# tanishqkumar/ssd

Hardware: NVIDIA H100
Metric: decode tokens/sec (sync speculative decoding, accept-len reported) (higher is better)
Workload: dtype bf16

## Files before the change

ssd_b200/csrc/draft_stream.cuh:

```cuda
#pragma once
#include "common.cuh"
#include "sampling.cuh"

namespace ssdk {

constexpr int kDsConsumers = 256;
constexpr int kDsWarps = kDsConsumers / 32;
constexpr int kDsThreads = kDsConsumers + 32;
constexpr int kDsMaxLayers = 32;
constexpr int kDsSplits = 16;
constexpr int kDsShortSplits = 8;
constexpr int kDsLongCtx = 256;
constexpr int kDsSlotBytes = 32768;
constexpr int kDsMaxSlots = 6;
constexpr int kDsMaxSteps = 8;
constexpr int kDsBtSmem = 32;

struct DsLayer {
  const __nv_bfloat16 *qkv, *o, *gate_up, *down, *in_norm, *post_norm, *q_norm, *k_norm;
};

struct DsParams {
  int d, L, H, KV, ffn, vocab, qk_norm;
  float eps, scale_log2;
  const __nv_bfloat16 *embed, *final_norm, *lm_head;
  const float* rope;
  __nv_bfloat16 *k_cache, *v_cache;
  long long cache_layer_stride;
  int block_size, max_blocks;
  int64_t* tok_buf;
  int n_fwd;
  int skip_last_head;
  const int32_t* ctx0;
  const int32_t* block_table;
  __nv_bfloat16 *vec_qkv, *vec_attn, *vec_o, *vec_act, *vec_down, *resid0, *resid1;
  float* attn_part;
  __nv_bfloat16* logits;
  long long logits_ld;
  const float* temp;
  const uint64_t* dyn;
  uint64_t seed, call_base;
  ArgMax* samp_partial;
  unsigned* bar_state;
  unsigned* attn_ticket;
  int n_slots;
  DsLayer layers[kDsMaxLayers];
  const int64_t* pend_tok;
  __nv_bfloat16* vec_row0;
};

struct DsVecs {
  __nv_bfloat16 *qkv, *attn, *o, *down, *resid0, *resid1, *act;
  SSDK_DEVINL __nv_bfloat16* resid(int i) const { return i ? resid1 : resid0; }
};
SSDK_DEVINL DsVecs ds_row0_vecs(const DsParams& p, int hd) {
  DsVecs v{};
  __nv_bfloat16* b = p.vec_row0;
  if (!b) return v;
  v.qkv = b; b += ((p.H + 2 * p.KV) * hd + 7) / 8 * 8;
  v.attn = b; b += p.H * hd;
  v.o = b; b += p.d;
  v.down = b; b += p.d;
  v.resid0 = b; b += p.d;
  v.resid1 = b; b += p.d;
  v.act = b;
  return v;
}
__host__ SSDK_DEVINL int ds_xs_floats(int d, int ffn, int q_width) {
  const int a = 2 * d > ffn ? 2 * d : ffn;
  return a > q_width ? a : q_width;
}

SSDK_DEVINL void ds_sync() {
#ifdef SSDK_HOST_EMU
  ::emu::named_barrier(1, kDsConsumers);
#else
  asm volatile("bar.sync 1, 256;" ::: "memory");
#endif
}

struct DsGridBar {
  unsigned long long* counter;
  unsigned long long target;
  __device__ void init() {
    if (threadIdx.x == 0) {
      const unsigned long long c = ld_relaxed_gpu_u64(counter);
      target = c - c % (unsigned long long)gridDim.x;
    }
  }
  __device__ void sync() {
    ds_sync();
    if (threadIdx.x == 0) {
      target += (unsigned long long)gridDim.x;
      red_add_release_gpu_u64(counter, 1ull);
      const long long t0 = clock64();
      while (ld_relaxed_gpu_u64(counter) < target) {
        if (clock64() - t0 > 4000000000LL) __trap();
      }
      fence_acq_rel_gpu();
    }
    ds_sync();
  }
};

SSDK_DEVINL uint4 ds_ldcg16(const void* p) { return __ldcg(reinterpret_cast<const uint4*>(p)); }
SSDK_DEVINL float2 ds_bf2(uint32_t w) { return __bfloat1622float2(*reinterpret_cast<const __nv_bfloat162*>(&w)); }

SSDK_DEVINL void ds_mark(int f, int point) {
  if (f == 1 && threadIdx.x == 0) trace_mark(64 + point);
}

enum { DS_QKV = 0, DS_O = 1, DS_GU = 2, DS_DOWN = 3, DS_HEAD = 4 };
enum { DS_PLAIN = 0, DS_PAIR = 1, DS_SPLIT = 2 };
struct DsGeom {
  int K;
  int rows;
  int kind;
  int rpj;
  int segs;
  int nj;
};
__host__ SSDK_DEVINL bool ds_geometry(int K, int rows, bool pair, DsGeom* g) {
  g->K = K; g->rows = rows; g->segs = 1;
  if (K < 256 || K > 8192 || (K % 256) != 0) return false;
  if (pair) {
    if (K > 2048) return false;
    g->kind = DS_PAIR; g->rpj = 8;
  } else if (K <= 2048) {
    g->kind = DS_PLAIN; g->rpj = 8;
  } else {
    g->kind = DS_SPLIT; g->rpj = K <= 4096 ? 4 : 2; g->segs = kDsWarps / g->rpj;
    if ((K % (256 * g->segs)) != 0) return false;
  }
  g->nj = (rows + g->rpj - 1) / g->rpj;
  return true;
}
SSDK_DEVINL bool ds_has_head(const DsParams& p, int f) { return !(p.skip_last_head && f == p.n_fwd - 1); }
SSDK_DEVINL const __nv_bfloat16* ds_weight(const DsParams& p, int l, int m) {
  const DsLayer& lw = p.layers[l < p.L ? l : 0];
  return m == DS_QKV ? lw.qkv : (m == DS_O ? lw.o : (m == DS_GU ? lw.gate_up : (m == DS_DOWN ? lw.down : p.lm_head)));
}

struct DsCursor {
  int f, l, m, s;
  bool valid;
};
SSDK_DEVINL void ds_cursor_settle(const DsParams& p, const DsGeom* geom, DsCursor& c) {
  while (c.valid && c.s >= geom[c.m].nj) {
    c.s = (int)blockIdx.x;
    if (c.m == DS_HEAD) {
      c.f++; c.l = 0; c.m = DS_QKV;
    } else if (c.m == DS_DOWN) {
      c.l++; c.m = DS_QKV;
      if (c.l == p.L) {
        if (ds_has_head(p, c.f)) c.m = DS_HEAD;
        else { c.f++; c.l = 0; }
      }
    } else {
      c.m++;
    }
    if (c.f >= p.n_fwd) c.valid = false;
  }
// ... 201 lines not shown
  for (int s = (int)blockIdx.x; s < g.nj; s += (int)gridDim.x, ++it) {
    const uint8_t* st = ds_acquire(ring, 0);
    const float acc = ds_dot_seg(st + w_off, steps, lane, xr);
    float acc0 = 0.f;
    if constexpr (TWO) acc0 = ds_dot_seg0(st + w_off, steps, lane, x0 + seg * seg_len);
    ds_release(ring, 0, lane);
    ring.taken += 1u;
    float* rb = res + (it & 1u) * kDsWarps;
    float* rb0 = rb + 2 * kDsWarps;
    if (lane == 0) {
      rb[warp] = acc;
      if constexpr (TWO) rb0[warp] = acc0;
    }
    ds_sync();
    if ((int)threadIdx.x < g.rpj) {
      const int row = s * g.rpj + (int)threadIdx.x;
      if (row < g.rows) {
        float v = 0.f;
        for (int q = 0; q < g.segs; ++q) v += rb[(int)threadIdx.x * g.segs + q];
        y[row] = f2bf(v);
        if constexpr (TWO) {
          float v0 = 0.f;
          for (int q = 0; q < g.segs; ++q) v0 += rb0[(int)threadIdx.x * g.segs + q];
          r0.y[row] = f2bf(v0);
        }
      }
    }
  }
}
SSDK_DEVINL void ds_consume(DsRing& ring, const DsGeom& g, float* xs, float* res, __nv_bfloat16* y, bool two,
                            const DsRow0& r0) {
  if (g.kind == DS_PLAIN) {
    if (two) ds_consume_plain<false, true>(ring, g, xs, y, nullptr, r0);
    else ds_consume_plain<false>(ring, g, xs, y, nullptr);
  } else {
    if (two) ds_consume_split<true>(ring, g, xs, res, y, r0);
    else ds_consume_split<false>(ring, g, xs, res, y, r0);
  }
}
SSDK_DEVINL void ds_consume_gu(DsRing& ring, const DsGeom& g, float* xs, __nv_bfloat16* act, bool two, const DsRow0& r0) {
  if (two) ds_consume_pair<true>(ring, g, xs, act, r0);
  else ds_consume_pair<false>(ring, g, xs, act, r0);
}

SSDK_DEVINL float ds_block_sum(float v, float* red) {
  const int lane = threadIdx.x & 31, wid = threadIdx.x >> 5;
  v = warp_sum(v);
  ds_sync();
  if (lane == 0) red[wid] = v;
  ds_sync();
  float t = (lane < kDsWarps) ? red[lane] : 0.f;
  return warp_sum(t);
}

struct DsPre {
  uint4 w, b;
};
SSDK_DEVINL DsPre ds_preload(const __nv_bfloat16* b, const __nv_bfloat16* w, int d) {
  DsPre r;
  const int i = threadIdx.x * 8;
  r.w = r.b = make_uint4(0u, 0u, 0u, 0u);
  if (i < d) {
    r.w = *reinterpret_cast<const uint4*>(w + i);
    if (b) r.b = ds_ldcg16(b + i);
  }
  return r;
}
SSDK_DEVINL void ds_norm_prologue(const __nv_bfloat16* a, const __nv_bfloat16* b, __nv_bfloat16* resid_out,
                                  const __nv_bfloat16* w, float eps, int d, float* xs, float* red, const DsPre* pre) {
  float ss = 0.f;
  const int i0 = threadIdx.x * 8;
  for (int i = i0; i < d; i += kDsConsumers * 8) {
    float x[8];
    unpack_bf16x8(ds_ldcg16(a + i), x);
    if (b) {
      float y[8];
      unpack_bf16x8((pre && i == i0) ? pre->b : ds_ldcg16(b + i), y);
#pragma unroll
      for (int j = 0; j < 8; ++j) x[j] += y[j];
    }
    if (resid_out && blockIdx.x == 0) *reinterpret_cast<uint4*>(resid_out + i) = pack_bf16x8(x);
#pragma unroll
    for (int j = 0; j < 8; ++j) {
      xs[i + j] = x[j];
      ss += x[j] * x[j];
    }
  }
  ss = ds_block_sum(ss, red);
  const float rstd = rsqrtf(ss / (float)d + eps);
  for (int i = i0; i < d; i += kDsConsumers * 8) {
    float wv[8];
    unpack_bf16x8((pre && i == i0) ? pre->w : *reinterpret_cast<const uint4*>(w + i), wv);
#pragma unroll
    for (int j = 0; j < 8; ++j) xs[i + j] = bf16_round(xs[i + j] * rstd * wv[j]);
  }
  ds_sync();
}
SSDK_DEVINL void ds_load_vec(const __nv_bfloat16* v, int n, float* xs) {
  for (int i = threadIdx.x * 8; i < n; i += kDsConsumers * 8) {
    float x[8];
    unpack_bf16x8(ds_ldcg16(v + i), x);
#pragma unroll
    for (int j = 0; j < 8; ++j) xs[i + j] = x[j];
  }
  ds_sync();
}

SSDK_DEVINL int ds_num_splits(int ctx) {
  return ctx > kDsLongCtx ? kDsSplits : min(kDsShortSplits, max(1, (ctx + 7) >> 3));
}
SSDK_DEVINL int ds_page_of(const DsParams& p, const int* bt_s, int t) {
  const int i = t / p.block_size;
  return p.max_blocks <= kDsBtSmem ? bt_s[i] : p.block_table[i];
}
template <int HD, int TB>
SSDK_DEVINL void ds_load_kv(const DsParams& p, const int* bt_s, const __nv_bfloat16* kbase, const __nv_bfloat16* vbase, int h,
                            int tb, int t1, int pos, int lane, float (&kv)[TB][HD / 32], float (&vv)[TB][HD / 32]) {
  constexpr int EPL = HD / 32;
  static_assert(EPL == 2 || EPL == 4, "head_dim 64 or 128");
#pragma unroll
  for (int u = 0; u < TB; ++u) {
    const int t = tb + u * kDsWarps;
#pragma unroll
    for (int e = 0; e < EPL; ++e) kv[u][e] = vv[u][e] = 0.f;
    if (t < t1 && t != pos) {
      const int blk = ds_page_of(p, bt_s, t);
      const size_t off = (((size_t)blk * p.block_size + t % p.block_size) * p.KV + h) * HD + lane * EPL;
      if constexpr (EPL == 2) {
        const float2 a = ds_bf2(__ldcg(reinterpret_cast<const uint32_t*>(kbase + off)));
        const float2 b = ds_bf2(__ldcg(reinterpret_cast<const uint32_t*>(vbase + off)));
        kv[u][0] = a.x; kv[u][1] = a.y; vv[u][0] = b.x; vv[u][1] = b.y;
      } else {
        const uint2 a = __ldcg(reinterpret_cast<const uint2*>(kbase + off));
        const uint2 b = __ldcg(reinterpret_cast<const uint2*>(vbase + off));
        float2 f = ds_bf2(a.x); kv[u][0] = f.x; kv[u][1] = f.y;
        f = ds_bf2(a.y); kv[u][EPL - 2] = f.x; kv[u][EPL - 1] = f.y;
        f = ds_bf2(b.x); vv[u][0] = f.x; vv[u][1] = f.y;
        f = ds_bf2(b.y); vv[u][EPL - 2] = f.x; vv[u][EPL - 1] = f.y;
      }
    }
  }
}
template <int HD, int GMAX, int TB>
SSDK_DEVINL void ds_attention_unit(const DsParams& p, const __nv_bfloat16* vqkv, __nv_bfloat16* vattn, int layer, int h,
                                   int s, int ns, int ctx, float* sm, int* flag, const int* bt_s) {
  constexpr int HALF = HD / 2;
  constexpr int EPL = HD / 32;
  const int warp = threadIdx.x >> 5, lane = threadIdx.x & 31;
  const int G = p.H / p.KV;
  const int pos = ctx - 1;
  float* sq = sm;
  float* sk = sq + GMAX * HD;
  float* sv = sk + HD;
  float* sred = sv + HD;

  const int per = (ctx + ns - 1) / ns;
  const int t0 = s * per, t1 = min(ctx, t0 + per);
  const __nv_bfloat16* kbase = p.k_cache + (size_t)layer * p.cache_layer_stride;
  const __nv_bfloat16* vbase = p.v_cache + (size_t)layer * p.cache_layer_stride;
  float kv[TB][EPL], vv[TB][EPL];
  ds_load_kv<HD, TB>(p, bt_s, kbase, vbase, h, t0 + warp, t1, pos, lane, kv, vv);

  const float* cs = p.rope + (size_t)pos * HD;
  for (int row = warp; row < G + 2; row += kDsWarps) {
    const int kind = row < G ? 0 : (row == G ? 1 : 2);
    const int col0 = (kind == 0 ? (h * G + row) : (kind == 1 ? p.H + h : p.H + p.KV + h)) * HD;
    float x1[(HALF + 31) / 32], x2[(HALF + 31) / 32];
    float ss = 0.f;
#pragma unroll
    for (int t = 0; t < (HALF + 31) / 32; ++t) {
      const int i = lane + 32 * t;
      x1[t] = x2[t] = 0.f;
      if (i < HALF) {
        const unsigned short a = __ldcg(reinterpret_cast<const unsigned short*>(vqkv + col0 + i));
        const unsigned short b = __ldcg(reinterpret_cast<const unsigned short*>(vqkv + col0 + HALF + i));
        x1[t] = __bfloat162float(__ushort_as_bfloat16(a));
        x2[t] = __bfloat162float(__ushort_as_bfloat16(b));
        ss += x1[t] * x1[t] + x2[t] * x2[t];
      }
    }
    float* dst = kind == 0 ? sq + row * HD : (kind == 1 ? sk : sv);
    if (kind == 2) {
#pragma unroll
      for (int t = 0; t < (HALF + 31) / 32; ++t) {
        const int i = lane + 32 * t;
        if (i < HALF) {
          dst[i] = x1[t];
          dst[HALF + i] = x2[t];
        }
      }
      continue;
    }
    const __nv_bfloat16* nw = p.qk_norm ? (kind == 0 ? p.layers[layer].q_norm : p.layers[layer].k_norm) : nullptr;
    if (nw) {
      ss = warp_sum(ss);
      const float rstd = rsqrtf(ss / (float)HD + p.eps);
#pragma unroll
      for (int t = 0; t < (HALF + 31) / 32; ++t) {
        const int i = lane + 32 * t;
        if (i < HALF) {
          x1[t] = bf16_round(x1[t] * rstd * bf2f(nw[i]));
          x2[t] = bf16_round(x2[t] * rstd * bf2f(nw[HALF + i]));
        }
      }
    }
#pragma unroll
    for (int t = 0; t < (HALF + 31) / 32; ++t) {
      const int i = lane + 32 * t;
      if (i < HALF) {
        const float c = cs[i], sn = cs[HALF + i];
        dst[i] = bf16_round(x1[t] * c - x2[t] * sn);
        dst[HALF + i] = bf16_round(x2[t] * c + x1[t] * sn);
      }
    }
  }
  ds_sync();

  const int blk_new = ds_page_of(p, bt_s, pos);
  if (s == 0 && blk_new >= 0) {
    const size_t slot = (size_t)blk_new * p.block_size + pos % p.block_size;
    __nv_bfloat16* kc = p.k_cache + (size_t)layer * p.cache_layer_stride + (slot * p.KV + h) * HD;
    __nv_bfloat16* vc = p.v_cache + (size_t)layer * p.cache_layer_stride + (slot * p.KV + h) * HD;
    for (int i = threadIdx.x; i < HD; i += kDsConsumers) {
      kc[i] = f2bf(sk[i]);
      vc[i] = f2bf(sv[i]);
    }
  }

  float qreg[GMAX][EPL];
#pragma unroll
  for (int g = 0; g < GMAX; ++g)
#pragma unroll
    for (int e = 0; e < EPL; ++e) qreg[g][e] = (g < G) ? sq[g * HD + lane * EPL + e] : 0.f;
  float m[GMAX], l[GMAX], acc[GMAX][EPL];
#pragma unroll
  for (int g = 0; g < GMAX; ++g) {
    m[g] = -INFINITY;
    l[g] = 0.f;
#pragma unroll
    for (int e = 0; e < EPL; ++e) acc[g][e] = 0.f;
  }
  for (int tb = t0 + warp; tb < t1; tb += TB * kDsWarps) {
    if (tb != t0 + warp) ds_load_kv<HD, TB>(p, bt_s, kbase, vbase, h, tb, t1, pos, lane, kv, vv);
#pragma unroll
    for (int u = 0; u < TB; ++u) {
      const int t = tb + u * kDsWarps;
      if (t < t1) {
        if (t == pos) {
#pragma unroll
          for (int e = 0; e < EPL; ++e) {
            kv[u][e] = sk[lane * EPL + e];
            vv[u][e] = sv[lane * EPL + e];
          }
        }
#pragma unroll
        for (int g = 0; g < GMAX; ++g) {
          if (g < G) {
            float sc = 0.f;
#pragma unroll
            for (int e = 0; e < EPL; ++e) sc = fmaf(qreg[g][e], kv[u][e], sc);
            sc = warp_sum(sc) * p.scale_log2;
            const float mn = fmaxf(m[g], sc);
            const float corr = exp2f(m[g] - mn);
            const float pr = exp2f(sc - mn);
            l[g] = l[g] * corr + pr;
#pragma unroll
            for (int e = 0; e < EPL; ++e) acc[g][e] = acc[g][e] * corr + pr * vv[u][e];
            m[g] = mn;
          }
        }
      }
    }
  }
  constexpr int LDR = HD + 2;
#pragma unroll
  for (int g = 0; g < GMAX; ++g) {
    if (g < G) {
      float* w = sred + ((size_t)warp * G + g) * LDR;
#pragma unroll
      for (int e = 0; e < EPL; ++e) w[lane * EPL + e] = acc[g][e];
      if (lane == 0) {
        w[HD] = m[g];
        w[HD + 1] = l[g];
      }
    }
  }
  ds_sync();
  for (int idx = threadIdx.x; idx < G * HD; idx += kDsConsumers) {
    const int g = idx / HD, dim = idx - g * HD;
    float mx = -INFINITY;
    for (int w = 0; w < kDsWarps; ++w) mx = fmaxf(mx, sred[((size_t)w * G + g) * LDR + HD]);
    float o = 0.f, ll = 0.f;
    if (mx != -INFINITY) {
      for (int w = 0; w < kDsWarps; ++w) {
        const float* r = sred + ((size_t)w * G + g) * LDR;
        const float wt = exp2f(r[HD] - mx);
        o += r[dim] * wt;
        ll += r[HD + 1] * wt;
      }
    }
    if (ns == 1) {
      vattn[(size_t)(h * G + g) * HD + dim] = f2bf(ll > 0.f ? o / ll : 0.f);
    } else {
      float* out = p.attn_part + ((size_t)(h * G + g) * kDsSplits + s) * LDR;
      out[dim] = o;
      if (dim == 0) {
        out[HD] = mx;
        out[HD + 1] = ll;
      }
    }
  }
  if (ns == 1) {
    ds_sync();
    return;
  }
  ds_sync();
  if (threadIdx.x == 0) *flag = (atom_add_acq_rel_gpu(p.attn_ticket + h, 1u) == (unsigned)ns - 1u) ? 1 : 0;
  ds_sync();
  if (*flag) {
    if (threadIdx.x == 0) st_relaxed_gpu_u32(p.attn_ticket + h, 0u);
    for (int idx = threadIdx.x; idx < G * HD; idx += kDsConsumers) {
      const int g = idx / HD, dim = idx - g * HD;
      const float* base = p.attn_part + (size_t)(h * G + g) * kDsSplits * LDR;
      float ms[kDsSplits], ls[kDsSplits], os[kDsSplits];
      float mx = -INFINITY;
#pragma unroll
      for (int q = 0; q < kDsSplits; ++q) {
        const bool on = q < ns;
        ms[q] = on ? __ldcg(base + q * LDR + HD) : -INFINITY;
        ls[q] = on ? __ldcg(base + q * LDR + HD + 1) : 0.f;
        os[q] = on ? __ldcg(base + q * LDR + dim) : 0.f;
        mx = fmaxf(mx, ms[q]);
      }
      float o = 0.f, l = 0.f;
#pragma unroll
      for (int q = 0; q < kDsSplits; ++q) {
        const float wt = (ms[q] == -INFINITY) ? 0.f : exp2f(ms[q] - mx);
        o += os[q] * wt;
        l += ls[q] * wt;
      }
      vattn[(size_t)(h * G + g) * HD + dim] = f2bf(l > 0.f ? o / l : 0.f);
    }
  }
  ds_sync();
}


template <int HD, int GMAX>
__global__ void __launch_bounds__(kDsThreads, 1) draft_stream_kernel(const __grid_constant__ DsParams p) {
  SSDK_DYN_SMEM(uint8_t, ds_smem);
  SSDK_STATIC_SMEM(uint64_t, full_bar, kDsMaxSlots);
  SSDK_STATIC_SMEM(uint64_t, empty_bar, kDsMaxSlots);
  SSDK_STATIC_SMEM(DsGeom, geom, 5);
  SSDK_STATIC_SMEM(float, red, 32);
  SSDK_STATIC_SMEM(float, res, 4 * kDsWarps);
  SSDK_STATIC_SMEM(ArgMax, ared, 32);
  SSDK_SHARED_VAR(int, tok_s);
  SSDK_SHARED_VAR(int, flag_s);
  SSDK_STATIC_SMEM(int, bt_s, kDsBtSmem);
  float* xs = reinterpret_cast<float*>(ds_smem + (size_t)p.n_slots * kDsSlotBytes);
  float* scratch = xs + ds_xs_floats(p.d, p.ffn, p.H * HD);
  if (threadIdx.x < kDsBtSmem && (int)threadIdx.x < p.max_blocks) bt_s[threadIdx.x] = p.block_table[threadIdx.x];
  if (threadIdx.x == 0) {
    trace_mark(TR_MISC);
    ds_geometry(p.d, (p.H + 2 * p.KV) * HD, false, &geom[DS_QKV]);
    ds_geometry(p.H * HD, p.d, false, &geom[DS_O]);
    ds_geometry(p.d, p.ffn, true, &geom[DS_GU]);
    ds_geometry(p.ffn, p.d, false, &geom[DS_DOWN]);
    ds_geometry(p.d, p.vocab, false, &geom[DS_HEAD]);
    for (int s = 0; s < p.n_slots; ++s) {
      mbar_init(&full_bar[s], 1);
      mbar_init(&empty_bar[s], kDsWarps);
    }
    fence_mbar_init();
  }
  __syncthreads();

  if (threadIdx.x >= kDsConsumers) {
    if (threadIdx.x == kDsConsumers) ds_producer(p, geom, ds_smem, full_bar, empty_bar);
    return;
  }

  DsRing ring;
  ring.base = ds_smem;
  ring.full = full_bar;
  ring.empty = empty_bar;
  ring.n_slots = (unsigned)p.n_slots;
  ring.taken = 0u;
  DsGridBar bar;
  bar.counter = reinterpret_cast<unsigned long long*>(p.bar_state);
  bar.target = 0;
  bar.init();

  const int ctx_base = p.ctx0[0];
  const float T = p.temp ? p.temp[0] : 0.f;
  const uint64_t seed = p.dyn ? p.dyn[0] : p.seed;
  const uint64_t call0 = p.dyn ? p.dyn[1] * 16ull : p.call_base;
  __nv_bfloat16* resid[2] = {p.resid0, p.resid1};
  long long tok = p.tok_buf[0];
  const long long tok0 = p.pend_tok ? p.pend_tok[0] : -1;
  const DsVecs v0 = ds_row0_vecs(p, HD);

  for (int f = 0; f < p.n_fwd; ++f) {
    if (threadIdx.x == 0 && f > 0) trace_mark(TR_MISC);
    const int ctx = ctx_base + f + 1;
    const __nv_bfloat16* emb = p.embed + (size_t)tok * p.d;
    const bool two = f == 0 && tok0 >= 0;
    int cur = 0;
    DsPre pre;
    for (int l = 0; l < p.L; ++l) {
      const DsLayer& lw = p.layers[l];
      if (l == 0) {
        if (two) ds_norm_prologue(p.embed + (size_t)tok0 * p.d, nullptr, v0.resid(cur ^ 1), lw.in_norm, p.eps, p.d, xs + p.d, red,
                                  nullptr);
        ds_norm_prologue(emb, nullptr, resid[cur ^ 1], lw.in_norm, p.eps, p.d, xs, red, nullptr);
      } else {
        if (two) ds_norm_prologue(v0.down, v0.resid(cur), v0.resid(cur ^ 1), lw.in_norm, p.eps, p.d, xs + p.d, red, nullptr);
        ds_norm_prologue(p.vec_down, resid[cur], resid[cur ^ 1], lw.in_norm, p.eps, p.d, xs, red, &pre);
      }
      cur ^= 1;
      ds_mark(f, 0);
      ds_consume(ring, geom[DS_QKV], xs, res, p.vec_qkv, two, DsRow0{xs + p.d, nullptr, v0.qkv});
      ds_mark(f, 1);
      bar.sync();
      ds_mark(f, 2);
#ifdef SSDK_TRACE_FINE
      bar.sync();
      ds_mark(f, 12);
#endif
      if (two) {
        const int ns0 = ds_num_splits(ctx - 1);
        for (int u = blockIdx.x; u < p.KV * ns0; u += gridDim.x) {
          if (ns0 == kDsSplits)
            ds_attention_unit<HD, GMAX, 8>(p, v0.qkv, v0.attn, l, u / ns0, u % ns0, ns0, ctx - 1, scratch, &flag_s, bt_s);
          else ds_attention_unit<HD, GMAX, 4>(p, v0.qkv, v0.attn, l, u / ns0, u % ns0, ns0, ctx - 1, scratch, &flag_s, bt_s);
        }
        bar.sync();
      }
      const int ns = ds_num_splits(ctx);
      for (int u = blockIdx.x; u < p.KV * ns; u += gridDim.x) {
        if (ns == kDsSplits)
          ds_attention_unit<HD, GMAX, 8>(p, p.vec_qkv, p.vec_attn, l, u / ns, u % ns, ns, ctx, scratch, &flag_s, bt_s);
        else ds_attention_unit<HD, GMAX, 4>(p, p.vec_qkv, p.vec_attn, l, u / ns, u % ns, ns, ctx, scratch, &flag_s, bt_s);
      }
      ds_mark(f, 3);
      bar.sync();
      ds_mark(f, 4);
      ds_load_vec(p.vec_attn, p.H * HD, xs);
      ds_consume(ring, geom[DS_O], xs, res, p.vec_o, two, DsRow0{nullptr, v0.attn, v0.o});
      ds_mark(f, 5);
      pre = ds_preload(resid[cur], lw.post_norm, p.d);
      bar.sync();
      ds_mark(f, 6);
      if (two) ds_norm_prologue(v0.o, v0.resid(cur), v0.resid(cur ^ 1), lw.post_norm, p.eps, p.d, xs + p.d, red, nullptr);
      ds_norm_prologue(p.vec_o, resid[cur], resid[cur ^ 1], lw.post_norm, p.eps, p.d, xs, red, &pre);
      cur ^= 1;
      ds_mark(f, 7);
      ds_consume_gu(ring, geom[DS_GU], xs, p.vec_act, two, DsRow0{xs + p.d, nullptr, v0.act});
      ds_mark(f, 8);
      bar.sync();
      ds_mark(f, 9);
      ds_load_vec(p.vec_act, p.ffn, xs);
      ds_consume(ring, geom[DS_DOWN], xs, res, p.vec_down, two, DsRow0{nullptr, v0.act, v0.down});
      ds_mark(f, 10);
      pre = ds_preload(resid[cur], l + 1 < p.L ? p.layers[l + 1].in_norm : p.final_norm, p.d);
      bar.sync();
      ds_mark(f, 11);
    }
    if (!ds_has_head(p, f)) break;
    ds_norm_prologue(p.vec_down, resid[cur], nullptr, p.final_norm, p.eps, p.d, xs, red, &pre);
    DsSample smp;
    smp.greedy = (T == 0.f);
    smp.invT = smp.greedy ? 1.f : 1.f / T;
    smp.seed = seed;
    smp.call_id = call0 + (uint64_t)f;
    smp.best = ArgMax{-INFINITY, 0x7fffffff};
    ds_consume_plain<true>(ring, geom[DS_HEAD], xs, p.logits ? p.logits + (size_t)f * p.logits_ld : nullptr, &smp);
    if ((threadIdx.x & 31) == 0) ared[threadIdx.x >> 5] = smp.best;
    ds_sync();
    if (threadIdx.x == 0) {
      ArgMax b = ared[0];
      for (int w = 1; w < kDsWarps; ++w) b = argmax_better(b, ared[w]);
      p.samp_partial[blockIdx.x] = b;
    }
    bar.sync();
    {
      ArgMax a{-INFINITY, 0x7fffffff};
      for (int i = threadIdx.x; i < (int)gridDim.x; i += kDsConsumers) {
        ArgMax q;
        q.v = __ldcg(&p.samp_partial[i].v);
        q.i = __ldcg(&p.samp_partial[i].i);
        a = argmax_better(a, q);
      }
      a = warp_argmax(a);
      ds_sync();
      if ((threadIdx.x & 31) == 0) ared[threadIdx.x >> 5] = a;
      ds_sync();
      if (threadIdx.x == 0) {
        ArgMax b = ared[0];
        for (int w = 1; w < kDsWarps; ++w) b = argmax_better(b, ared[w]);
        tok_s = b.i;
      }
      ds_sync();
      tok = tok_s;
      if (blockIdx.x == 0 && threadIdx.x == 0) p.tok_buf[f + 1] = tok;
    }
  }
}

}
```

ssd_b200/csrc/engine.cu:

```cuda
#include <cuda.h>
#include <cuda_runtime.h>
#include <cudaTypedefs.h>
#include <nccl.h>

#include <algorithm>
#include <cstdarg>
#include <cstdio>
#include <cstdlib>
#include <cstring>
#include <map>
#include <string>
#include <tuple>
#include <vector>

#include "../../include/ssdk.h"
#include "attention.cuh"
#include "common.cuh"
#include "elementwise.cuh"
#include "gemm.cuh"
#include "sampling.cuh"
#include "draft_stream.cuh"

using namespace ssdk;
typedef __nv_bfloat16 bf16;
// ... 331 lines not shown
      return (size_t)S * kMaxTokens * N;
    };
    part = std::max(part, need(m.qkv_dim, m.d));
    part = std::max(part, need(m.d, m.H * m.hd));
    part = std::max(part, need(2 * m.ffn, m.d));
    part = std::max(part, need(m.d, m.ffn));
  }
  Workspace scratch_ws;
  Workspace& w = base ? e->ws : scratch_ws;
  const int K = e->rt.spec_k, MB = e->rt.max_batch;
  w.hidden = (bf16*)take((size_t)kMaxTokens * dmax * 2);
  w.residual = (bf16*)take((size_t)kMaxTokens * dmax * 2);
  w.q = (bf16*)take((size_t)kMaxTokens * Hmax * hdmax * 2);
  w.attn_out = (bf16*)take((size_t)kMaxTokens * Hmax * hdmax * 2);
  w.act = (bf16*)take((size_t)kMaxTokens * fmax * 2);
  w.last_hidden = (bf16*)take((size_t)kMaxTokens * dmax * 2);
  w.dense_tmp = (bf16*)take((size_t)kMaxTokens * std::max(dmax, qmax) * 2);
  w.partials = (float*)take(part * 4);
  w.partial_floats = part;
  w.att_o = (float*)take((size_t)kMaxTokens * Hmax * kAttnMaxSplit * hdmax * 4);
  w.att_lse = (float*)take((size_t)kMaxTokens * Hmax * kAttnMaxSplit * 4);
  w.att_counters = (unsigned*)take((size_t)kMaxTokens * 64 * 4);
  w.ar_state = (unsigned*)take(64);
  w.pub_counters = (unsigned*)take(512 * 4);
  w.positions = (int64_t*)take(kMaxTokens * 8);
  w.slot_mapping = (int32_t*)take(kMaxTokens * 4);
  w.context_lens = (int32_t*)take(kMaxTokens * 4);
  w.out_dev = take(e->out_bytes);
  w.tok_buf = (int64_t*)w.out_dev;
  w.n_accept = (int32_t*)(w.out_dev ? w.out_dev + e->off_out_nacc : nullptr);
  w.recovery = (int64_t*)(w.out_dev ? w.out_dev + e->off_out_rec : nullptr);
  w.log_tokens = (int64_t*)take((size_t)MB * kLogCap * 8);
  w.log_len = (int32_t*)take((size_t)MB * 4);
  w.ids_in = (int64_t*)take(kFwInBytes);
  w.var_cu_q = (int32_t*)(w.ids_in ? (uint8_t*)w.ids_in + kFwInCuOff : nullptr);
  w.var_tiles = (AttnTile*)(w.ids_in ? (uint8_t*)w.ids_in + kFwInTileOff : nullptr);
  w.out_tok = (int64_t*)take(kMaxTokens * 8);
  w.logits_q = (bf16*)take((size_t)MB * std::max(K, 1) * vmax * 2);
  w.logits_p = (bf16*)take((size_t)MB * (K + 1) * vmax * 2);
  w.logits_last = (bf16*)take((size_t)kMaxTokens * vmax * 2);
  w.logits_shard = (bf16*)take((size_t)kMaxTokens * vmax * 2);
  w.logits_gather = (bf16*)take((size_t)kMaxTokens * vmax * 2);
  w.step_dev = take(e->step_bytes);
  w.samp_partial = (ArgMax*)take((size_t)kMaxTokens * kSampleChunks * sizeof(ArgMax));
  w.samp_counters = (unsigned*)take(kMaxTokens * 4);
  w.ver_rows = (RowPart*)take((size_t)kVerifyMaxRows * kVerifyCtas * sizeof(RowPart));
  w.ver_rec = (RecPart*)take((size_t)kVerifyMaxBatch * kVerifyCtas * sizeof(RecPart));
  w.ver_counters = (unsigned*)take(64);
  const size_t ds_elems = ds_vec_elems(qmax, dmax, fmax, Hmax * hdmax);
  w.ds_vec = (bf16*)take(ds_elems * 2);
  w.ds_vec0 = (bf16*)take(ds_elems * 2);
  w.fold_ids = (int64_t*)take((size_t)MB * 2 * 8);
  w.ds_attn = (float*)take((size_t)Hmax * kDsSplits * (hdmax + 2) * 4);
  w.ds_sync = (unsigned*)take(256);
  return (int64_t)align_up(off, 1024);
}

struct VarlenFwd {
  AttnVarlen attn;
  AttnPlan plan;
  int n_tiles;
  int M;
};
struct Fwd {
  int which;
  int B, Q;
  const int64_t* ids;
  int ids_stride;
  const int32_t* ctx0;
  const int32_t* block_tables;
  int pos_offset;
  int logits_mode;
  bf16* logits_out;
  int64_t logits_ld;
  const VarlenFwd* var = nullptr;
  const int64_t* pend = nullptr;
};

static int attn_plan_raw(int H, int KV, int B, int Q, int max_ctx, int* TQ, int* MT, int* nqt, int* nsplit) {
  AttnPlan pl;
  const int rc = attn_make_plan(H, KV, B, Q, max_ctx, num_sms(), &pl);
  if (rc == 1) return fail("unsupported GQA ratio %d/%d", H, KV);
  if (rc != 0) return fail("attention tile too large");
  *TQ = pl.TQ;
  *MT = pl.MT;
  *nqt = pl.n_qtiles;
  *nsplit = pl.n_split;
  return 0;
}
static int attn_plan(const Model& m, int B, int Q, int* TQ, int* MT, int* nqt, int* nsplit, int max_ctx) {
  return attn_plan_raw(m.H, m.KV, B, Q, max_ctx, TQ, MT, nqt, nsplit);
}

template <int HD, int MT>
static int launch_attn_inst(Launcher& L, const AttnParams& p, const AttnVarlen* var, dim3 grid) {
  const size_t smem = (size_t)2 * 2 * kAttChunk * (HD + 8) * 2;
  static bool attr_set = false;
  if (!attr_set) {
    CK(cudaFuncSetAttribute(paged_attn_kernel<HD, MT>, cudaFuncAttributeMaxDynamicSharedMemorySize, (int)smem));
    CK(cudaFuncSetAttribute(paged_attn_varlen_kernel<HD, MT>, cudaFuncAttributeMaxDynamicSharedMemorySize, (int)smem));
    attr_set = true;
  }
  if (var) return L.go(paged_attn_varlen_kernel<HD, MT>, grid, dim3(attn_warps(MT) * 32), smem, p, *var);
  return L.go(paged_attn_kernel<HD, MT>, grid, dim3(attn_warps(MT) * 32), smem, p);
}
static int launch_attn(Launcher& L, const AttnParams& p, const AttnVarlen* var, int hd, int MT, dim3 grid) {
  if (hd == 128 && MT == 1) return launch_attn_inst<128, 1>(L, p, var, grid);
// ... 357 lines not shown
  pdl_launch_dependents();
  pdl_wait();
  const int b = threadIdx.x;
  if (b < B) {
    const int n = n_accept[b] + 1;
    int len = log_len[b];
    for (int j = 0; j < n && len < log_cap; ++j) log_tokens[(size_t)b * log_cap + len++] = tok_buf[(size_t)b * Kp1 + j];
    log_len[b] = len;
    ctx[b] += n;
    recovery_in[b] = recovery_out[b];
    pend[b] = (n == Kp1) ? tok_buf[(size_t)b * Kp1 + Kp1 - 1] : -1;
  }
  if (threadIdx.x == 0) seed_step[1] += 1;
}

static bool draft_stream_enabled() {
  static int v = -1;
  if (v < 0) v = env_int("SSDK_DRAFT_STREAM", 1) != 0 ? 1 : 0;
  return v == 1;
}
constexpr int kMaxDynSmem = 227 * 1024 - 2048;
static size_t ds_fixed_smem(const Model& m) {
  const int G = m.H / m.KV, gmax = G <= 4 ? 4 : 8;
  const size_t xs = (size_t)ds_xs_floats(m.d, m.ffn, m.H * m.hd);
  const size_t scratch = (size_t)gmax * m.hd + 2 * m.hd + (size_t)kDsWarps * gmax * (m.hd + 2);
  return (xs + scratch) * 4 + 256;
}
static int ds_ring_slots(const Model& m) {
  const size_t fixed = ds_fixed_smem(m);
  if (fixed + 3 * (size_t)kDsSlotBytes > (size_t)kMaxDynSmem) return 0;
  return (int)std::min<size_t>(kDsMaxSlots, ((size_t)kMaxDynSmem - fixed) / kDsSlotBytes);
}
static bool draft_stream_supported(const Model& m, int B) {
  const int G = m.KV ? m.H / m.KV : 0;
  DsGeom g;
  return B == 1 && m.cfg.tp_size == 1 && m.cfg.layers <= kDsMaxLayers && (m.hd == 64 || m.hd == 128) && G >= 1 && G <= 8 &&
         m.H % m.KV == 0 && m.KV <= 32 && m.d % 8 == 0 && (m.H * m.hd) % 8 == 0 && m.ffn % 8 == 0 &&
         ds_geometry(m.d, m.qkv_dim, false, &g) && ds_geometry(m.H * m.hd, m.d, false, &g) &&
         ds_geometry(m.d, m.ffn, true, &g) && ds_geometry(m.ffn, m.d, false, &g) && ds_geometry(m.d, m.cfg.vocab, false, &g) &&
         ds_ring_slots(m) >= 3;
}
static int draft_stream_max_ctx() {
  static int v = -1;
  if (v < 0) v = std::max(0, env_int("SSDK_DRAFT_STREAM_MAX_CTX", 1024));
  return v;
}
static bool use_draft_stream(ssdk_engine* e, int B, int ctx_bound) {
  const Model& drf = e->model[SSDK_DRAFT];
  return drf.present && draft_stream_enabled() && draft_stream_supported(drf, B) &&
         ctx_bound + e->rt.spec_k + 1 <= draft_stream_max_ctx();
}
template <int HD, int GMAX>
static int launch_draft_stream(Launcher& L, const DsParams& p, size_t smem) {
  static bool attr_set = false;
  if (!attr_set) {
    CK(cudaFuncSetAttribute(draft_stream_kernel<HD, GMAX>, cudaFuncAttributeMaxDynamicSharedMemorySize, (int)smem));
    attr_set = true;
  }
  cudaLaunchConfig_t cfg = {};
  cfg.gridDim = dim3(num_sms());
  cfg.blockDim = dim3(kDsThreads);
  cfg.dynamicSmemBytes = smem;
  cfg.stream = L.st;
  cudaLaunchAttribute attr[1];
  attr[0].id = cudaLaunchAttributeCooperative;
  attr[0].val.cooperative = 1;
  cfg.attrs = attr;
  cfg.numAttrs = 1;
  cudaError_t err = cudaLaunchKernelEx(&cfg, draft_stream_kernel<HD, GMAX>, p);
  if (err != cudaSuccess) return fail("draft stream launch failed: %s", cudaGetErrorString(err));
  L.barrier_op();
  ++L.count;
  return 0;
}
static int enqueue_draft_stream(ssdk_engine* e, Launcher& L, int64_t* tok_buf, int n_fwd, const int64_t* pend,
                                const int32_t* ctx0, const int32_t* block_table, const float* temp, const uint64_t* dyn,
                                bf16* logits, int64_t logits_ld) {
  Model& m = e->model[SSDK_DRAFT];
  Workspace& w = e->ws;
  DsParams p;
  memset(&p, 0, sizeof(p));
  p.d = m.d; p.L = m.cfg.layers; p.H = m.H; p.KV = m.KV; p.ffn = m.ffn; p.vocab = m.cfg.vocab; p.qk_norm = m.cfg.qk_norm;
  p.eps = m.cfg.rms_eps;
  p.scale_log2 = (1.0f / sqrtf((float)m.hd)) * 1.4426950408889634f;
  p.embed = m.embed.ptr; p.final_norm = m.final_norm; p.lm_head = m.lm_head.ptr; p.rope = m.rope;
  p.k_cache = m.k_cache; p.v_cache = m.v_cache;
  p.cache_layer_stride = (long long)m.num_blocks * e->rt.block_size * m.KV * m.hd;
  p.block_size = e->rt.block_size; p.max_blocks = e->rt.max_blocks_per_seq;
  p.tok_buf = tok_buf; p.n_fwd = n_fwd; p.skip_last_head = 0;
  p.pend_tok = pend; p.vec_row0 = w.ds_vec0;
  p.ctx0 = ctx0; p.block_table = block_table;
  bf16* v = w.ds_vec;
  p.vec_qkv = v; v += align_up((size_t)m.qkv_dim, 8);
  p.vec_attn = v; v += (size_t)m.H * m.hd;
  p.vec_o = v; v += m.d;
  p.vec_down = v; v += m.d;
  p.resid0 = v; v += m.d;
  p.resid1 = v; v += m.d;
  p.vec_act = v;
  p.attn_part = w.ds_attn;
  p.logits = logits; p.logits_ld = logits_ld;
  p.temp = temp; p.dyn = dyn;
  p.samp_partial = w.samp_partial;
  p.bar_state = w.ds_sync;
  p.attn_ticket = w.ds_sync + 8;
  p.n_slots = ds_ring_slots(m);
  for (int l = 0; l < p.L; ++l) {
    const LayerW& lw = m.layers[l];
    p.layers[l] = DsLayer{lw.qkv.ptr, lw.o.ptr, lw.gate_up.ptr, lw.down.ptr, lw.input_norm, lw.post_norm, lw.q_norm, lw.k_norm};
  }
// ... 872 lines not shown
```

Measured before the change: 377.4.

## Fuse two-row draft attention into one phase and batch dual RMSNorm reductions

In the first draft step, where two token rows are processed, attention for both rows now runs in one combined work loop, removing a grid-wide barrier between them. The second row folds in the first row's fresh K/V from shared memory rather than reading it from cache, and each row gets separate partial buffers and tickets. The two RMSNorm prologues are merged into one pass with a single paired block reduction, which cuts block-level syncs. The cost is a larger partial-attention workspace and more complex attention indexing, plus extra trace markers.

```diff
diff --git a/ssd_b200/csrc/draft_stream.cuh b/ssd_b200/csrc/draft_stream.cuh
--- a/ssd_b200/csrc/draft_stream.cuh
+++ b/ssd_b200/csrc/draft_stream.cuh
@@ -8,7 +8,8 @@
 constexpr int kDsWarps = kDsConsumers / 32;
 constexpr int kDsThreads = kDsConsumers + 32;
 constexpr int kDsMaxLayers = 32;
-constexpr int kDsSplits = 16;
+constexpr int kDsMaxSplits = 16;
+constexpr int kDsSplits = 2 * kDsMaxSplits;
 constexpr int kDsShortSplits = 8;
 constexpr int kDsLongCtx = 256;
 constexpr int kDsSlotBytes = 32768;
@@ -106,8 +107,9 @@
 SSDK_DEVINL uint4 ds_ldcg16(const void* p) { return __ldcg(reinterpret_cast<const uint4*>(p)); }
 SSDK_DEVINL float2 ds_bf2(uint32_t w) { return __bfloat1622float2(*reinterpret_cast<const __nv_bfloat162*>(&w)); }
 
-SSDK_DEVINL void ds_mark(int f, int point) {
-  if (f == 1 && threadIdx.x == 0) trace_mark(64 + point);
+enum { DSM_HEAD = 13, DSM_TOKEN = 14, DSM_START = 15 };
+SSDK_DEVINL void ds_mark(int f, bool two, int point) {
+  if (f <= 1 && threadIdx.x == 0) trace_mark((f == 1 ? 64 : (two ? 96 : 80)) + point);
 }
 
 enum { DS_QKV = 0, DS_O = 1, DS_GU = 2, DS_DOWN = 3, DS_HEAD = 4 };
@@ -415,6 +417,20 @@
   float t = (lane < kDsWarps) ? red[lane] : 0.f;
   return warp_sum(t);
 }
+SSDK_DEVINL float2 ds_block_sum2(float v0, float v1, float* red) {
+  const int lane = threadIdx.x & 31, wid = threadIdx.x >> 5;
+  v0 = warp_sum(v0);
+  v1 = warp_sum(v1);
+  ds_sync();
+  if (lane == 0) {
+    red[wid] = v0;
+    red[kDsWarps + wid] = v1;
+  }
+  ds_sync();
+  const float t0 = (lane < kDsWarps) ? red[lane] : 0.f;
+  const float t1 = (lane < kDsWarps) ? red[kDsWarps + lane] : 0.f;
+  return make_float2(warp_sum(t0), warp_sum(t1));
+}
 
 struct DsPre {
   uint4 w, b;
@@ -429,8 +445,8 @@
   }
   return r;
 }
-SSDK_DEVINL void ds_norm_prologue(const __nv_bfloat16* a, const __nv_bfloat16* b, __nv_bfloat16* resid_out,
-                                  const __nv_bfloat16* w, float eps, int d, float* xs, float* red, const DsPre* pre) {
+SSDK_DEVINL float ds_norm_load(const __nv_bfloat16* a, const __nv_bfloat16* b, __nv_bfloat16* resid_out, int d, float* xs,
+                               const uint4* pb) {
   float ss = 0.f;
   const int i0 = threadIdx.x * 8;
   for (int i = i0; i < d; i += kDsConsumers * 8) {
@@ -438,7 +454,7 @@
     unpack_bf16x8(ds_ldcg16(a + i), x);
     if (b) {
       float y[8];
-      unpack_bf16x8((pre && i == i0) ? pre->b : ds_ldcg16(b + i), y);
+      unpack_bf16x8((pb && i == i0) ? *pb : ds_ldcg16(b + i), y);
 #pragma unroll
       for (int j = 0; j < 8; ++j) x[j] += y[j];
     }
@@ -449,14 +465,33 @@
       ss += x[j] * x[j];
     }
   }
-  ss = ds_block_sum(ss, red);
-  const float rstd = rsqrtf(ss / (float)d + eps);
+  return ss;
+}
+SSDK_DEVINL void ds_norm_scale(const __nv_bfloat16* w, float rstd, int d, float* xs, const uint4* pw) {
+  const int i0 = threadIdx.x * 8;
   for (int i = i0; i < d; i += kDsConsumers * 8) {
     float wv[8];
-    unpack_bf16x8((pre && i == i0) ? pre->w : *reinterpret_cast<const uint4*>(w + i), wv);
+    unpack_bf16x8((pw && i == i0) ? *pw : *reinterpret_cast<const uint4*>(w + i), wv);
 #pragma unroll
     for (int j = 0; j < 8; ++j) xs[i + j] = bf16_round(xs[i + j] * rstd * wv[j]);
   }
+}
+SSDK_DEVINL void ds_norm_prologue(const __nv_bfloat16* a, const __nv_bfloat16* b, __nv_bfloat16* resid_out,
+                                  const __nv_bfloat16* w, float eps, int d, float* xs, float* red, const DsPre* pre) {
+  float ss = ds_norm_load(a, b, resid_out, d, xs, pre ? &pre->b : nullptr);
+  ss = ds_block_sum(ss, red);
+  ds_norm_scale(w, rsqrtf(ss / (float)d + eps), d, xs, pre ? &pre->w : nullptr);
+  ds_sync();
+}
+SSDK_DEVINL void ds_norm_prologue2(const __nv_bfloat16* a, const __nv_bfloat16* b, __nv_bfloat16* resid_out,
+                                   const __nv_bfloat16* a0, const __nv_bfloat16* b0, __nv_bfloat16* resid_out0,
+                                   const __nv_bfloat16* w, float eps, int d, float* xs, float* xs0, float* red,
+                                   const DsPre* pre) {
+  const float ss0 = ds_norm_load(a0, b0, resid_out0, d, xs0, nullptr);
+  const float ss1 = ds_norm_load(a, b, resid_out, d, xs, pre ? &pre->b : nullptr);
+  const float2 ss = ds_block_sum2(ss0, ss1, red);
+  ds_norm_scale(w, rsqrtf(ss.x / (float)d + eps), d, xs0, pre ? &pre->w : nullptr);
+  ds_norm_scale(w, rsqrtf(ss.y / (float)d + eps), d, xs, pre ? &pre->w : nullptr);
   ds_sync();
 }
 SSDK_DEVINL void ds_load_vec(const __nv_bfloat16* v, int n, float* xs) {
@@ -470,7 +505,7 @@
 }
 
 SSDK_DEVINL int ds_num_splits(int ctx) {
-  return ctx > kDsLongCtx ? kDsSplits : min(kDsShortSplits, max(1, (ctx + 7) >> 3));
+  return ctx > kDsLongCtx ? kDsMaxSplits : min(kDsShortSplits, max(1, (ctx + 7) >> 3));
 }
 SSDK_DEVINL int ds_page_of(const DsParams& p, const int* bt_s, int t) {
   const int i = t / p.block_size;
@@ -478,7 +513,7 @@
 }
 template <int HD, int TB>
 SSDK_DEVINL void ds_load_kv(const DsParams& p, const int* bt_s, const __nv_bfloat16* kbase, const __nv_bfloat16* vbase, int h,
-                            int tb, int t1, int pos, int lane, float (&kv)[TB][HD / 32], float (&vv)[TB][HD / 32]) {
+                            int tb, int t1, int tsm, int lane, float (&kv)[TB][HD / 32], float (&vv)[TB][HD / 32]) {
   constexpr int EPL = HD / 32;
   static_assert(EPL == 2 || EPL == 4, "head_dim 64 or 128");
 #pragma unroll
@@ -486,7 +521,7 @@
     const int t = tb + u * kDsWarps;
 #pragma unroll
     for (int e = 0; e < EPL; ++e) kv[u][e] = vv[u][e] = 0.f;
-    if (t < t1 && t != pos) {
+    if (t < t1 && t < tsm) {
       const int blk = ds_page_of(p, bt_s, t);
       const size_t off = (((size_t)blk * p.block_size + t % p.block_size) * p.KV + h) * HD + lane * EPL;
       if constexpr (EPL == 2) {
@@ -504,14 +539,22 @@
     }
   }
 }
+struct DsAttnRow {
+  const __nv_bfloat16* qkv;
+  __nv_bfloat16* attn;
+  float* part;
+  unsigned* ticket;
+};
 template <int HD, int GMAX, int TB>
-SSDK_DEVINL void ds_attention_unit(const DsParams& p, const __nv_bfloat16* vqkv, __nv_bfloat16* vattn, int layer, int h,
-                                   int s, int ns, int ctx, float* sm, int* flag, const int* bt_s) {
+SSDK_DEVINL void ds_attention_unit(const DsParams& p, const DsAttnRow& r, const __nv_bfloat16* qkv_prev, int layer, int h,
+                                   int s, int ns, int ctx, float* sm, float* sprev, int* flag, const int* bt_s) {
   constexpr int HALF = HD / 2;
   constexpr int EPL = HD / 32;
   const int warp = threadIdx.x >> 5, lane = threadIdx.x & 31;
   const int G = p.H / p.KV;
   const int pos = ctx - 1;
+  const bool has_prev = qkv_prev != nullptr;
+  const int tsm = has_prev ? pos - 1 : pos;
   float* sq = sm;
   float* sk = sq + GMAX * HD;
   float* sv = sk + HD;
@@ -522,12 +565,15 @@
   const __nv_bfloat16* kbase = p.k_cache + (size_t)layer * p.cache_layer_stride;
   const __nv_bfloat16* vbase = p.v_cache + (size_t)layer * p.cache_layer_stride;
   float kv[TB][EPL], vv[TB][EPL];
-  ds_load_kv<HD, TB>(p, bt_s, kbase, vbase, h, t0 + warp, t1, pos, lane, kv, vv);
+  ds_load_kv<HD, TB>(p, bt_s, kbase, vbase, h, t0 + warp, t1, tsm, lane, kv, vv);
 
   const float* cs = p.rope + (size_t)pos * HD;
-  for (int row = warp; row < G + 2; row += kDsWarps) {
-    const int kind = row < G ? 0 : (row == G ? 1 : 2);
-    const int col0 = (kind == 0 ? (h * G + row) : (kind == 1 ? p.H + h : p.H + p.KV + h)) * HD;
+  for (int row = warp; row < G + (has_prev ? 4 : 2); row += kDsWarps) {
+    const bool prev = row >= G + 2;
+    const int rw = prev ? row - 2 : row;
+    const int kind = rw < G ? 0 : (rw == G ? 1 : 2);
+    const int col0 = (kind == 0 ? (h * G + rw) : (kind == 1 ? p.H + h : p.H + p.KV + h)) * HD;
+    const __nv_bfloat16* vqkv = prev ? qkv_prev : r.qkv;
     float x1[(HALF + 31) / 32], x2[(HALF + 31) / 32];
     float ss = 0.f;
 #pragma unroll
@@ -542,7 +588,7 @@
         ss += x1[t] * x1[t] + x2[t] * x2[t];
       }
     }
-    float* dst = kind == 0 ? sq + row * HD : (kind == 1 ? sk : sv);
+    float* dst = kind == 0 ? sq + rw * HD : (kind == 1 ? (prev ? sprev : sk) : (prev ? sprev + HD : sv));
     if (kind == 2) {
 #pragma unroll
       for (int t = 0; t < (HALF + 31) / 32; ++t) {
@@ -567,11 +613,12 @@
         }
       }
     }
+    const float* csr = prev ? cs - HD : cs;
 #pragma unroll
     for (int t = 0; t < (HALF + 31) / 32; ++t) {
       const int i = lane + 32 * t;
       if (i < HALF) {
-        const float c = cs[i], sn = cs[HALF + i];
+        const float c = csr[i], sn = csr[HALF + i];
         dst[i] = bf16_round(x1[t] * c - x2[t] * sn);
         dst[HALF + i] = bf16_round(x2[t] * c + x1[t] * sn);
       }
@@ -604,16 +651,18 @@
     for (int e = 0; e < EPL; ++e) acc[g][e] = 0.f;
   }
   for (int tb = t0 + warp; tb < t1; tb += TB * kDsWarps) {
-    if (tb != t0 + warp) ds_load_kv<HD, TB>(p, bt_s, kbase, vbase, h, tb, t1, pos, lane, kv, vv);
+    if (tb != t0 + warp) ds_load_kv<HD, TB>(p, bt_s, kbase, vbase, h, tb, t1, tsm, lane, kv, vv);
 #pragma unroll
     for (int u = 0; u < TB; ++u) {
       const int t = tb + u * kDsWarps;
       if (t < t1) {
-        if (t == pos) {
+        if (t >= tsm) {
+          const float* nk = t == pos ? sk : sprev;
+          const float* nv = t == pos ? sv : sprev + HD;
 #pragma unroll
           for (int e = 0; e < EPL; ++e) {
-            kv[u][e] = sk[lane * EPL + e];
-            vv[u][e] = sv[lane * EPL + e];
+            kv[u][e] = nk[lane * EPL + e];
+            vv[u][e] = nv[lane * EPL + e];
           }
         }
 #pragma unroll
@@ -656,16 +705,16 @@
     float o = 0.f, ll = 0.f;
     if (mx != -INFINITY) {
       for (int w = 0; w < kDsWarps; ++w) {
-        const float* r = sred + ((size_t)w * G + g) * LDR;
-        const float wt = exp2f(r[HD] - mx);
-        o += r[dim] * wt;
-        ll += r[HD + 1] * wt;
+        const float* pw = sred + ((size_t)w * G + g) * LDR;
+        const float wt = exp2f(pw[HD] - mx);
+        o += pw[dim] * wt;
+        ll += pw[HD + 1] * wt;
       }
     }
     if (ns == 1) {
-      vattn[(size_t)(h * G + g) * HD + dim] = f2bf(ll > 0.f ? o / ll : 0.f);
+      r.attn[(size_t)(h * G + g) * HD + dim] = f2bf(ll > 0.f ? o / ll : 0.f);
     } else {
-      float* out = p.attn_part + ((size_t)(h * G + g) * kDsSplits + s) * LDR;
+      float* out = r.part + ((size_t)(h * G + g) * kDsMaxSplits + s) * LDR;
       out[dim] = o;
       if (dim == 0) {
         out[HD] = mx;
@@ -678,17 +727,17 @@
     return;
   }
   ds_sync();
-  if (threadIdx.x == 0) *flag = (atom_add_acq_rel_gpu(p.attn_ticket + h, 1u) == (unsigned)ns - 1u) ? 1 : 0;
+  if (threadIdx.x == 0) *flag = (atom_add_acq_rel_gpu(r.ticket + h, 1u) == (unsigned)ns - 1u) ? 1 : 0;
   ds_sync();
   if (*flag) {
-    if (threadIdx.x == 0) st_relaxed_gpu_u32(p.attn_ticket + h, 0u);
+    if (threadIdx.x == 0) st_relaxed_gpu_u32(r.ticket + h, 0u);
     for (int idx = threadIdx.x; idx < G * HD; idx += kDsConsumers) {
       const int g = idx / HD, dim = idx - g * HD;
-      const float* base = p.attn_part + (size_t)(h * G + g) * kDsSplits * LDR;
-      float ms[kDsSplits], ls[kDsSplits], os[kDsSplits];
+      const float* base = r.part + (size_t)(h * G + g) * kDsMaxSplits * LDR;
+      float ms[kDsMaxSplits], ls[kDsMaxSplits], os[kDsMaxSplits];
       float mx = -INFINITY;
 #pragma unroll
-      for (int q = 0; q < kDsSplits; ++q) {
+      for (int q = 0; q < kDsMaxSplits; ++q) {
         const bool on = q < ns;
         ms[q] = on ? __ldcg(base + q * LDR + HD) : -INFINITY;
         ls[q] = on ? __ldcg(base + q * LDR + HD + 1) : 0.f;
@@ -697,12 +746,12 @@
       }
       float o = 0.f, l = 0.f;
 #pragma unroll
-      for (int q = 0; q < kDsSplits; ++q) {
+      for (int q = 0; q < kDsMaxSplits; ++q) {
         const float wt = (ms[q] == -INFINITY) ? 0.f : exp2f(ms[q] - mx);
         o += os[q] * wt;
         l += ls[q] * wt;
       }
-      vattn[(size_t)(h * G + g) * HD + dim] = f2bf(l > 0.f ? o / l : 0.f);
+      r.attn[(size_t)(h * G + g) * HD + dim] = f2bf(l > 0.f ? o / l : 0.f);
     }
   }
   ds_sync();
@@ -769,66 +818,68 @@
     const int ctx = ctx_base + f + 1;
     const __nv_bfloat16* emb = p.embed + (size_t)tok * p.d;
     const bool two = f == 0 && tok0 >= 0;
+    ds_mark(f, two, DSM_START);
     int cur = 0;
     DsPre pre;
     for (int l = 0; l < p.L; ++l) {
       const DsLayer& lw = p.layers[l];
       if (l == 0) {
-        if (two) ds_norm_prologue(p.embed + (size_t)tok0 * p.d, nullptr, v0.resid(cur ^ 1), lw.in_norm, p.eps, p.d, xs + p.d, red,
-                                  nullptr);
-        ds_norm_prologue(emb, nullptr, resid[cur ^ 1], lw.in_norm, p.eps, p.d, xs, red, nullptr);
+        if (two)
+          ds_norm_prologue2(emb, nullptr, resid[cur ^ 1], p.embed + (size_t)tok0 * p.d, nullptr, v0.resid(cur ^ 1), lw.in_norm,
+                            p.eps, p.d, xs, xs + p.d, red, nullptr);
+        else ds_norm_prologue(emb, nullptr, resid[cur ^ 1], lw.in_norm, p.eps, p.d, xs, red, nullptr);
       } else {
-        if (two) ds_norm_prologue(v0.down, v0.resid(cur), v0.resid(cur ^ 1), lw.in_norm, p.eps, p.d, xs + p.d, red, nullptr);
-        ds_norm_prologue(p.vec_down, resid[cur], resid[cur ^ 1], lw.in_norm, p.eps, p.d, xs, red, &pre);
+        if (two)
+          ds_norm_prologue2(p.vec_down, resid[cur], resid[cur ^ 1], v0.down, v0.resid(cur), v0.resid(cur ^ 1), lw.in_norm, p.eps,
+                            p.d, xs, xs + p.d, red, &pre);
+        else ds_norm_prologue(p.vec_down, resid[cur], resid[cur ^ 1], lw.in_norm, p.eps, p.d, xs, red, &pre);
       }
       cur ^= 1;
-      ds_mark(f, 0);
+      ds_mark(f, two, 0);
       ds_consume(ring, geom[DS_QKV], xs, res, p.vec_qkv, two, DsRow0{xs + p.d, nullptr, v0.qkv});
-      ds_mark(f, 1);
+      ds_mark(f, two, 1);
       bar.sync();
-      ds_mark(f, 2);
+      ds_mark(f, two, 2);
 #ifdef SSDK_TRACE_FINE
       bar.sync();
-      ds_mark(f, 12);
+      ds_mark(f, two, 12);
 #endif
-      if (two) {
-        const int ns0 = ds_num_splits(ctx - 1);
-        for (int u = blockIdx.x; u < p.KV * ns0; u += gridDim.x) {
-          if (ns0 == kDsSplits)
-            ds_attention_unit<HD, GMAX, 8>(p, v0.qkv, v0.attn, l, u / ns0, u % ns0, ns0, ctx - 1, scratch, &flag_s, bt_s);
-          else ds_attention_unit<HD, GMAX, 4>(p, v0.qkv, v0.attn, l, u / ns0, u % ns0, ns0, ctx - 1, scratch, &flag_s, bt_s);
-        }
-        bar.sync();
-      }
-      const int ns = ds_num_splits(ctx);
-      for (int u = blockIdx.x; u < p.KV * ns; u += gridDim.x) {
-        if (ns == kDsSplits)
-          ds_attention_unit<HD, GMAX, 8>(p, p.vec_qkv, p.vec_attn, l, u / ns, u % ns, ns, ctx, scratch, &flag_s, bt_s);
-        else ds_attention_unit<HD, GMAX, 4>(p, p.vec_qkv, p.vec_attn, l, u / ns, u % ns, ns, ctx, scratch, &flag_s, bt_s);
-      }
-      ds_mark(f, 3);
+      const int ns = ds_num_splits(ctx), ns0 = two ? ds_num_splits(ctx - 1) : 0;
+      for (int u = blockIdx.x; u < p.KV * (ns0 + ns); u += gridDim.x) {
+        const bool row0 = u < p.KV * ns0;
+        const int v = row0 ? u : u - p.KV * ns0, n = row0 ? ns0 : ns;
+        const DsAttnRow r = row0 ? DsAttnRow{v0.qkv, v0.attn, p.attn_part + (size_t)p.H * kDsMaxSplits * (HD + 2), p.attn_ticket + p.KV}
+                                 : DsAttnRow{p.vec_qkv, p.vec_attn, p.attn_part, p.attn_ticket};
+        const __nv_bfloat16* prev = (two && !row0) ? v0.qkv : nullptr;
+        if (n == kDsMaxSplits)
+          ds_attention_unit<HD, GMAX, 8>(p, r, prev, l, v / n, v % n, n, row0 ? ctx - 1 : ctx, scratch, xs, &flag_s, bt_s);
+        else ds_attention_unit<HD, GMAX, 4>(p, r, prev, l, v / n, v % n, n, row0 ? ctx - 1 : ctx, scratch, xs, &flag_s, bt_s);
+      }
+      ds_mark(f, two, 3);
       bar.sync();
-      ds_mark(f, 4);
+      ds_mark(f, two, 4);
       ds_load_vec(p.vec_attn, p.H * HD, xs);
       ds_consume(ring, geom[DS_O], xs, res, p.vec_o, two, DsRow0{nullptr, v0.attn, v0.o});
-      ds_mark(f, 5);
+      ds_mark(f, two, 5);
       pre = ds_preload(resid[cur], lw.post_norm, p.d);
       bar.sync();
-      ds_mark(f, 6);
-      if (two) ds_norm_prologue(v0.o, v0.resid(cur), v0.resid(cur ^ 1), lw.post_norm, p.eps, p.d, xs + p.d, red, nullptr);
-      ds_norm_prologue(p.vec_o, resid[cur], resid[cur ^ 1], lw.post_norm, p.eps, p.d, xs, red, &pre);
+      ds_mark(f, two, 6);
+      if (two)
+        ds_norm_prologue2(p.vec_o, resid[cur], resid[cur ^ 1], v0.o, v0.resid(cur), v0.resid(cur ^ 1), lw.post_norm, p.eps, p.d,
+                          xs, xs + p.d, red, &pre);
+      else ds_norm_prologue(p.vec_o, resid[cur], resid[cur ^ 1], lw.post_norm, p.eps, p.d, xs, red, &pre);
       cur ^= 1;
-      ds_mark(f, 7);
+      ds_mark(f, two, 7);
       ds_consume_gu(ring, geom[DS_GU], xs, p.vec_act, two, DsRow0{xs + p.d, nullptr, v0.act});
-      ds_mark(f, 8);
+      ds_mark(f, two, 8);
       bar.sync();
-      ds_mark(f, 9);
+      ds_mark(f, two, 9);
       ds_load_vec(p.vec_act, p.ffn, xs);
       ds_consume(ring, geom[DS_DOWN], xs, res, p.vec_down, two, DsRow0{nullptr, v0.act, v0.down});
-      ds_mark(f, 10);
+      ds_mark(f, two, 10);
       pre = ds_preload(resid[cur], l + 1 < p.L ? p.layers[l + 1].in_norm : p.final_norm, p.d);
       bar.sync();
-      ds_mark(f, 11);
+      ds_mark(f, two, 11);
     }
     if (!ds_has_head(p, f)) break;
     ds_norm_prologue(p.vec_down, resid[cur], nullptr, p.final_norm, p.eps, p.d, xs, red, &pre);
@@ -839,6 +890,7 @@
     smp.call_id = call0 + (uint64_t)f;
     smp.best = ArgMax{-INFINITY, 0x7fffffff};
     ds_consume_plain<true>(ring, geom[DS_HEAD], xs, p.logits ? p.logits + (size_t)f * p.logits_ld : nullptr, &smp);
+    ds_mark(f, two, DSM_HEAD);
     if ((threadIdx.x & 31) == 0) ared[threadIdx.x >> 5] = smp.best;
     ds_sync();
     if (threadIdx.x == 0) {
@@ -868,7 +920,8 @@
       tok = tok_s;
       if (blockIdx.x == 0 && threadIdx.x == 0) p.tok_buf[f + 1] = tok;
     }
-  }
-}
-
-}
+    ds_mark(f, two, DSM_TOKEN);
+  }
+}
+
+}
diff --git a/ssd_b200/csrc/engine.cu b/ssd_b200/csrc/engine.cu
--- a/ssd_b200/csrc/engine.cu
+++ b/ssd_b200/csrc/engine.cu
@@ -407,7 +407,7 @@
   w.ds_vec0 = (bf16*)take(ds_elems * 2);
   w.fold_ids = (int64_t*)take((size_t)MB * 2 * 8);
   w.ds_attn = (float*)take((size_t)Hmax * kDsSplits * (hdmax + 2) * 4);
-  w.ds_sync = (unsigned*)take(256);
+  w.ds_sync = (unsigned*)take(512);
   return (int64_t)align_up(off, 1024);
 }
 
@@ -871,10 +871,10 @@
 }
 template <int HD, int GMAX>
 static int launch_draft_stream(Launcher& L, const DsParams& p, size_t smem) {
-  static bool attr_set = false;
-  if (!attr_set) {
+  static size_t attr_smem = 0;
+  if (smem > attr_smem) {
     CK(cudaFuncSetAttribute(draft_stream_kernel<HD, GMAX>, cudaFuncAttributeMaxDynamicSharedMemorySize, (int)smem));
-    attr_set = true;
+    attr_smem = smem;
   }
   cudaLaunchConfig_t cfg = {};
   cfg.gridDim = dim3(num_sms());
```

After: 380.1 (median of 6 runs). No clear change (+0.7%).
